# microsoft/VidTok

Hardware: NVIDIA H100
Metric: frames/sec encode+decode, kl_causal_488 17x256x256 (higher is better)
Workload: dtype bf16

## Files before the change

vidtok_b200/csrc/tblock_tc.cu:

```cuda
#include <cuda.h>

#include <cstdio>
#include <cstdlib>
#include <cstring>
#include <string>

#include "common.cuh"
#include "kernels.h"
#include "tc_ptx.cuh"

namespace vt {

namespace {
using namespace tcx;

thread_local std::string g_tb_err;
constexpr int kC = 128;
constexpr int kKc = kC / 64;
constexpr uint32_t kTile = 128 * 128;
constexpr int kHSlots = 3;
constexpr int kConsumerWarps = 8;
constexpr int kProducerWarp = kConsumerWarps;
constexpr int kThreadsTb = (kConsumerWarps + 4) * 32;

struct TbParams {
  int B, T, H, W;
  int BW, BH;
  int tilesW, tilesH;
  long long num_strips;
  int stages;
  const float* bias1;
  const float* bias2;
  const float* g2;
  const float* b2;
  int ln_out, ln_out_silu;
  const float* g3;
  const float* b3;
  const bf16* x;
  bf16* out;
  bf16* out2;
  const bf16* n1;
  int cached_in;
  const bf16* cn1_in;
  const bf16* ch_in;
  bf16* cn1_out;
  bf16* ch_out;
};
struct TbMaps {
  CUtensorMap n1, w1, w2, cn1;
};

__device__ __forceinline__ float quad_sum(float v) {
  v += __shfl_xor_sync(0xffffffffu, v, 1);
  v += __shfl_xor_sync(0xffffffffu, v, 2);
  return v;
}

template <bool kCache>
__global__ void __launch_bounds__(kThreadsTb, 1) tblock_tc_kernel(const __grid_constant__ TbMaps maps, const TbParams p) {
  extern __shared__ uint8_t smem_raw[];
  const uint32_t smem_base = (smem_u32(smem_raw) + 1023u) & ~1023u;
  uint8_t* smem_gen = smem_raw + (smem_base - smem_u32(smem_raw));
  const int warp = threadIdx.x >> 5, lane = threadIdx.x & 31;
  const uint32_t h_base = smem_base;
  const uint32_t ring_base = h_base + kHSlots * kKc * kTile;
  const uint32_t stage_bytes = 2u * kTile;
  const uint32_t bar_base = ring_base + (uint32_t)p.stages * stage_bytes;
  auto full_bar = [&](int s) { return bar_base + 8u * s; };
  auto empty_bar = [&](int s) { return bar_base + 8u * (p.stages + s); };
  float* cst = reinterpret_cast<float*>(smem_gen + (bar_base - smem_base) + 16u * p.stages);

  for (int i = threadIdx.x; i < kC; i += kThreadsTb) {
    cst[i] = p.bias1 ? p.bias1[i] : 0.f;
    cst[kC + i] = 0.5f * p.g2[i];
    cst[2 * kC + i] = 0.5f * p.b2[i];
    cst[3 * kC + i] = p.bias2 ? p.bias2[i] : 0.f;
    const float sc = p.ln_out_silu ? 0.5f : 1.0f;
    cst[4 * kC + i] = p.ln_out ? sc * p.g3[i] : 0.f;
    cst[5 * kC + i] = p.ln_out ? sc * p.b3[i] : 0.f;
  }
  if (threadIdx.x == 0) {
    for (int s = 0; s < p.stages; ++s) { mbar_init(full_bar(s), 1); mbar_init(empty_bar(s), kConsumerWarps); }
    asm volatile("fence.mbarrier_init.release.cluster;" ::: "memory");
  }
  __syncthreads();

  if (warp >= kProducerWarp) {
    asm volatile("setmaxnreg.dec.sync.aligned.u32 40;" ::: "memory");
    if (warp != kProducerWarp) return;
    const bool el = elect_one();
    if (el) { prefetch_tmap(&maps.n1); prefetch_tmap(&maps.w1); prefetch_tmap(&maps.w2); }
    const bool front = kCache && p.cached_in;
    int stage = 0;
    uint32_t phase = 0;
    auto acquire = [&](uint32_t bytes) {
      mbar_wait(empty_bar(stage), phase ^ 1u);
      if (el) mbar_expect_tx(full_bar(stage), bytes);
    };
    auto advance = [&]() { if (++stage == p.stages) { stage = 0; phase ^= 1u; } };
    for (long long strip = blockIdx.x; strip < p.num_strips; strip += gridDim.x) {
      const int tw = (int)(strip % p.tilesW);
      const int th = (int)((strip / p.tilesW) % p.tilesH);
      const int b = (int)(strip / ((long long)p.tilesW * p.tilesH));
      const int w0 = tw * p.BW, h0 = th * p.BH;
      for (int t = 0; t < p.T; ++t) {
        for (int a = 0; a < 3; ++a) {
          const int tv = t - 2 + a;
          if (tv < 0 && !front) continue;
          for (int kc = 0; kc < kKc; ++kc) {
            acquire(2u * kTile);
            if (el) {
              const uint32_t sa = ring_base + stage * stage_bytes;
              if (kCache && tv < 0) tma_load_5d(sa, &maps.cn1, full_bar(stage), kc * 64, w0, h0, tv + 2, b);
              else tma_load_5d(sa, &maps.n1, full_bar(stage), kc * 64, w0, h0, tv, b);
              tma_load_3d(sa + kTile, &maps.w1, full_bar(stage), a * kC + kc * 64, 0, 0);
            }
            advance();
          }
        }
        for (int a = 0; a < 3; ++a) {
          if (t - 2 + a < 0 && !front) continue;
          for (int kc = 0; kc < kKc; ++kc) {
            acquire(kTile);
            if (el) tma_load_3d(ring_base + stage * stage_bytes + kTile, &maps.w2, full_bar(stage), a * kC + kc * 64, 0, 0);
            advance();
          }
        }
      }
    }
    return;
  }

  asm volatile("setmaxnreg.inc.sync.aligned.u32 232;" ::: "memory");
  const int g = warp >> 2, wq = warp & 3;
  const uint32_t hi = desc_hi(1024u);
  float acc[kC / 2];
  int stage = 0, pend_stage = -1;
  uint32_t phase = 0;
  auto release = [&]() {
    if (lane == 0 && pend_stage >= 0) mbar_arrive(empty_bar(pend_stage));
    pend_stage = -1;
  };
  auto kstep = [&](bool a_from_stage, uint32_t h_addr, uint32_t scale) {
    mbar_wait(full_bar(stage), phase);
    const uint32_t sa = ring_base + stage * stage_bytes;
    const uint32_t al = desc_lo(a_from_stage ? sa + (uint32_t)g * 64u * 128u : h_addr), bl = desc_lo(sa + kTile);
    wgmma_fence();
#pragma unroll
    for (uint32_t j = 0; j < 4u; ++j) wgmma_k16<kC, false>(acc, desc(al + 2u * j, hi), desc(bl + 2u * j, hi), j == 0 ? scale : 1u);
    wgmma_commit();
    wgmma_wait<1>();
    release();
    pend_stage = stage;
    if (++stage == p.stages) { stage = 0; phase ^= 1u; }
  };
  auto finish = [&]() {
    wgmma_wait<0>();
    acc_fence(acc);
    release();
  };
  auto wg_sync = [&]() { asm volatile("bar.sync %0, 128;" ::"r"(1 + g) : "memory"); };
  const float* bias1 = cst;
  const float* g2 = cst + kC;
  const float* b2 = cst + 2 * kC;
  const float* bias2 = cst + 3 * kC;
  const float* g3 = cst + 4 * kC;
  const float* b3 = cst + 5 * kC;
  const int cq = 2 * (lane & 3);
  const int rbase = 64 * g + 16 * wq + (lane >> 2);
  const bool front = kCache && p.cached_in;
  const int gtid = threadIdx.x & 127;
  auto slot_of = [&](int tv) { return h_base + (uint32_t)((tv + kHSlots) % kHSlots) * kKc * kTile; };
  auto ring_unit = [&](uint32_t slot, int row, int c) {
    return reinterpret_cast<uint4*>(smem_gen + (slot - smem_base) + (c >> 6) * kTile + row * 128 + ((((c & 63) >> 3) ^ (row & 7)) << 4));
  };

  for (long long strip = blockIdx.x; strip < p.num_strips; strip += gridDim.x) {
    const int tw = (int)(strip % p.tilesW);
    const int th = (int)((strip / p.tilesW) % p.tilesH);
    const int b = (int)(strip / ((long long)p.tilesW * p.tilesH));
    long long pos0[2];
#pragma unroll
    for (int r = 0; r < 2; ++r) {
      const int row = rbase + 8 * r;
      const int h = th * p.BH + row / p.BW, w = tw * p.BW + row % p.BW;
      pos0[r] = (((long long)b * p.T) * p.H + h) * p.W + w;
    }
    const long long frame = (long long)p.H * p.W;
    auto cache_pos = [&](int i, int j, int& row) {
      row = 64 * g + (i >> 4);
      const int h = th * p.BH + row / p.BW, w = tw * p.BW + row % p.BW;
      return ((((long long)b * 2 + j) * p.H + h) * p.W + w) * kC + (i & 15) * 8;
    };
    if (front) {
      wg_sync();
      for (int j = 0; j < 2; ++j)
        for (int i = gtid; i < 64 * 16; i += 128) {
          int row;
          const long long off = cache_pos(i, j, row);
          *ring_unit(slot_of(j - 2), row, (i & 15) * 8) = *reinterpret_cast<const uint4*>(p.ch_in + off);
        }
      fence_async_smem();
      wg_sync();
    }
    for (int t = 0; t < p.T; ++t) {
      uint32_t scale = 0;
      for (int a = 0; a < 3; ++a) {
        if (t - 2 + a < 0 && !front) continue;
        for (int kc = 0; kc < kKc; ++kc) { kstep(true, 0u, scale); scale = 1; }
      }
      finish();
      wg_sync();
      const uint32_t slot = h_base + (uint32_t)(t % kHSlots) * kKc * kTile;
#pragma unroll
      for (int r = 0; r < 2; ++r) {
        float s = 0.f, q = 0.f;
#pragma unroll
        for (int j = 0; j < kC / 8; ++j) {
          const int c = 8 * j + cq;
          const float f0 = acc[4 * j + 2 * r] + bias1[c], f1 = acc[4 * j + 2 * r + 1] + bias1[c + 1];
          s += f0 + f1;
          q = fmaf(f0, f0, q);
          q = fmaf(f1, f1, q);
          const uint32_t kp = pack_bf16x2(f0, f1);
          acc[4 * j + 2 * r] = bf16_lo(kp);
          acc[4 * j + 2 * r + 1] = bf16_hi(kp);
        }
        const float mean = quad_sum(s) * (1.0f / kC);
        float var = fmaf(-mean, mean, quad_sum(q) * (1.0f / kC));
        var = var < 0.f ? 0.f : var;
        const float rstd = rsqrtf(var + 1e-6f);
        const float nmr = -mean * rstd;
        const int row = rbase + 8 * r;
        uint8_t* hrow = smem_gen + (slot - smem_base) + row * 128;
#pragma unroll
        for (int j = 0; j < kC / 8; ++j) {
          const int c = 8 * j + cq;
          float y0 = fmaf(fmaf(acc[4 * j + 2 * r], rstd, nmr), g2[c], b2[c]);
          float y1 = fmaf(fmaf(acc[4 * j + 2 * r + 1], rstd, nmr), g2[c + 1], b2[c + 1]);
          y0 = fmaf(y0, tanh_approx(y0), y0);
          y1 = fmaf(y1, tanh_approx(y1), y1);
          const int cc = c & 63, u = cc >> 3;
          *reinterpret_cast<uint32_t*>(hrow + (c >> 6) * kTile + ((u ^ (row & 7)) << 4) + (cc & 7) * 2) = pack_bf16x2(y0, y1);
        }
      }
      fence_async_smem();
      wg_sync();
      scale = 0;
      for (int a = 0; a < 3; ++a) {
        const int tv = t - 2 + a;
        if (tv < 0 && !front) continue;
        const uint32_t hs = (kCache ? slot_of(tv) : h_base + (uint32_t)(tv % kHSlots) * kKc * kTile) + (uint32_t)g * 64u * 128u;
        for (int kc = 0; kc < kKc; ++kc) { kstep(false, hs + (uint32_t)kc * kTile, scale); scale = 1; }
      }
      finish();
#pragma unroll
      for (int r = 0; r < 2; ++r) {
        const long long off = (pos0[r] + (long long)t * frame) * kC;
        const bf16* xr = p.x + off;
        bf16* orow = p.out + off;
        float s = 0.f, q = 0.f;
#pragma unroll
        for (int j = 0; j < kC / 8; ++j) {
          const int c = 8 * j + cq;
          const uint32_t xw = *reinterpret_cast<const uint32_t*>(xr + c);
          const float f0 = acc[4 * j + 2 * r] + bias2[c] + bf16_lo(xw), f1 = acc[4 * j + 2 * r + 1] + bias2[c + 1] + bf16_hi(xw);
          s += f0 + f1;
          q = fmaf(f0, f0, q);
          q = fmaf(f1, f1, q);
          const uint32_t kp = pack_bf16x2(f0, f1);
          *reinterpret_cast<uint32_t*>(orow + c) = kp;
          acc[4 * j + 2 * r] = bf16_lo(kp);
          acc[4 * j + 2 * r + 1] = bf16_hi(kp);
        }
        if (!p.ln_out) continue;
        const float mean = quad_sum(s) * (1.0f / kC);
        float var = fmaf(-mean, mean, quad_sum(q) * (1.0f / kC));
        var = var < 0.f ? 0.f : var;
        const float rstd = rsqrtf(var + 1e-6f);
        const float nmr = -mean * rstd;
        bf16* o2 = p.out2 + off;
#pragma unroll
        for (int j = 0; j < kC / 8; ++j) {
          const int c = 8 * j + cq;
          float y0 = fmaf(fmaf(acc[4 * j + 2 * r], rstd, nmr), g3[c], b3[c]);
          float y1 = fmaf(fmaf(acc[4 * j + 2 * r + 1], rstd, nmr), g3[c + 1], b3[c + 1]);
          if (p.ln_out_silu) {
            y0 = fmaf(y0, tanh_approx(y0), y0);
            y1 = fmaf(y1, tanh_approx(y1), y1);
          }
          *reinterpret_cast<uint32_t*>(o2 + c) = pack_bf16x2(y0, y1);
        }
      }
    }
    if (kCache) {
      for (int j = 0; j < 2; ++j) {
        const int tv = p.T - 2 + j;
        for (int i = gtid; i < 64 * 16; i += 128) {
          int row;
          const long long off = cache_pos(i, j, row);
          const long long pix = off - (((long long)b * 2 + j) * frame) * kC;
          uint4 hv = make_uint4(0u, 0u, 0u, 0u), nv = hv;
          if (tv >= 0 || front) hv = *ring_unit(slot_of(tv), row, (i & 15) * 8);
          if (tv >= 0) nv = *reinterpret_cast<const uint4*>(p.n1 + (((long long)b * p.T + tv) * frame) * kC + pix);
          else if (front) nv = *reinterpret_cast<const uint4*>(p.cn1_in + (((long long)b * 2 + tv + 2) * frame) * kC + pix);
          *reinterpret_cast<uint4*>(p.ch_out + off) = hv;
          *reinterpret_cast<uint4*>(p.cn1_out + off) = nv;
        }
      }
    }
  }
}

typedef CUresult (*EncodeTiledFn)(CUtensorMap*, CUtensorMapDataType, cuuint32_t, void*, const cuuint64_t*,
                                  const cuuint64_t*, const cuuint32_t*, const cuuint32_t*, CUtensorMapInterleave,
                                  CUtensorMapSwizzle, CUtensorMapL2promotion, CUtensorMapFloatOOBfill);
EncodeTiledFn tb_get_encode() {
  static EncodeTiledFn fn = nullptr;
  static bool tried = false;
  if (!tried) {
    tried = true;
    void* f = nullptr;
    cudaDriverEntryPointQueryResult q;
    if (cudaGetDriverEntryPoint("cuTensorMapEncodeTiled", &f, cudaEnableDefault, &q) == cudaSuccess && q == cudaDriverEntryPointSuccess)
      fn = (EncodeTiledFn)f;
  }
  return fn;
}

bool strip_box(int H, int W, int& BW, int& BH) {
  for (int bw = 128; bw >= 1; bw >>= 1) {
    if (W % bw != 0) continue;
    const int bh = 128 / bw;
    if (bh <= 256 && H % bh == 0) { BW = bw; BH = bh; return true; }
  }
  return false;
}
}

const char* tblock_tc_last_error() { return g_tb_err.c_str(); }

bool tblock_tc_supported(int B, int T, int H, int W, int C, bool planning) {
  g_tb_err.clear();
  static int env = -1;
  if (env < 0) { const char* e = getenv("VT_TBLOCK"); env = e ? atoi(e) : 1; }
  if (!env) { g_tb_err = "disabled (VT_TBLOCK=0)"; return false; }
  if (C != kC) { g_tb_err = "C != 128"; return false; }
  if (B <= 0 || T <= 0) { g_tb_err = "empty"; return false; }
  int BW, BH;
  if (!strip_box(H, W, BW, BH)) { g_tb_err = "H x W not tileable by a 128-position box"; return false; }
  if (!planning && !tb_get_encode()) { g_tb_err = "cuTensorMapEncodeTiled unavailable"; return false; }
  return true;
}

cudaError_t launch_tblock_tc(const bf16* n1, const bf16* x, const bf16* w1, const float* bias1, const float* gamma2,
                             const float* beta2, const bf16* w2, const float* bias2, bf16* out, bf16* out2,
                             const float* gamma_out, const float* beta_out, bool out_silu, int B, int T, int H, int W,
                             cudaStream_t s, const TbCache* cache) {
  g_tb_err.clear();
  EncodeTiledFn enc = tb_get_encode();
  if (!enc) { g_tb_err = "cuTensorMapEncodeTiled unavailable"; return cudaErrorNotSupported; }
  TbParams p;
  memset(&p, 0, sizeof(p));
  if (!strip_box(H, W, p.BW, p.BH)) { g_tb_err = "H x W not tileable"; return cudaErrorInvalidValue; }
  p.B = B; p.T = T; p.H = H; p.W = W;
  p.tilesW = W / p.BW; p.tilesH = H / p.BH;
  p.num_strips = (long long)B * p.tilesH * p.tilesW;
  p.bias1 = bias1; p.bias2 = bias2; p.g2 = gamma2; p.b2 = beta2;
  p.ln_out = (out2 && gamma_out && beta_out) ? 1 : 0;
  p.ln_out_silu = out_silu ? 1 : 0;
  p.g3 = gamma_out; p.b3 = beta_out;
  p.x = x; p.out = out; p.out2 = out2;
  if (cache) {
    if (!cache->n1_out || !cache->h_out || (!cache->n1_in != !cache->h_in)) { g_tb_err = "cache: both outputs, and both or no inputs"; return cudaErrorInvalidValue; }
    p.n1 = n1;
    p.cached_in = cache->n1_in ? 1 : 0;
    p.cn1_in = cache->n1_in; p.ch_in = cache->h_in; p.cn1_out = cache->n1_out; p.ch_out = cache->h_out;
  }
  const size_t fixed = 1024 + (size_t)kHSlots * kKc * kTile + 6 * kC * 4;
  const size_t budget = 225 * 1024;
  int stages = (int)((budget - fixed) / (2 * kTile + 16));
  if (stages > 4) stages = 4;
  p.stages = stages;
  const size_t smem = fixed + (size_t)stages * (2 * kTile + 16);
  TbMaps maps;
  {
    cuuint64_t dims[5] = {(cuuint64_t)kC, (cuuint64_t)W, (cuuint64_t)H, (cuuint64_t)T, (cuuint64_t)B};
    cuuint64_t strides[4] = {(cuuint64_t)kC * 2, (cuuint64_t)W * kC * 2, (cuuint64_t)H * W * kC * 2, (cuuint64_t)T * H * W * kC * 2};
    cuuint32_t box[5] = {64, (cuuint32_t)p.BW, (cuuint32_t)p.BH, 1, 1};
    cuuint32_t es[5] = {1, 1, 1, 1, 1};
    CUresult r = enc(&maps.n1, CU_TENSOR_MAP_DATA_TYPE_BFLOAT16, 5, const_cast<bf16*>(n1), dims, strides, box, es, CU_TENSOR_MAP_INTERLEAVE_NONE,
                     CU_TENSOR_MAP_SWIZZLE_128B, CU_TENSOR_MAP_L2_PROMOTION_L2_256B, CU_TENSOR_MAP_FLOAT_OOB_FILL_NONE);
    if (r != CUDA_SUCCESS) { g_tb_err = "cuTensorMapEncodeTiled(n1) failed: " + std::to_string((int)r); return cudaErrorInvalidValue; }
    maps.cn1 = maps.n1;
    if (p.cached_in) {
      dims[3] = 2;
      strides[3] = 2ull * H * W * kC * 2;
      r = enc(&maps.cn1, CU_TENSOR_MAP_DATA_TYPE_BFLOAT16, 5, const_cast<bf16*>(p.cn1_in), dims, strides, box, es, CU_TENSOR_MAP_INTERLEAVE_NONE,
              CU_TENSOR_MAP_SWIZZLE_128B, CU_TENSOR_MAP_L2_PROMOTION_L2_256B, CU_TENSOR_MAP_FLOAT_OOB_FILL_NONE);
      if (r != CUDA_SUCCESS) { g_tb_err = "cuTensorMapEncodeTiled(n1 cache) failed: " + std::to_string((int)r); return cudaErrorInvalidValue; }
    }
  }
  for (int i = 0; i < 2; ++i) {
    cuuint64_t dims[3] = {(cuuint64_t)(3 * kC), (cuuint64_t)kC, 1};
    cuuint64_t strides[2] = {(cuuint64_t)(3 * kC) * 2, (cuuint64_t)(3 * kC) * kC * 2};
    cuuint32_t box[3] = {64, (cuuint32_t)kC, 1};
    cuuint32_t es[3] = {1, 1, 1};
    CUresult r = enc(i ? &maps.w2 : &maps.w1, CU_TENSOR_MAP_DATA_TYPE_BFLOAT16, 3, const_cast<bf16*>(i ? w2 : w1), dims, strides, box, es,
                     CU_TENSOR_MAP_INTERLEAVE_NONE, CU_TENSOR_MAP_SWIZZLE_128B, CU_TENSOR_MAP_L2_PROMOTION_L2_256B,
                     CU_TENSOR_MAP_FLOAT_OOB_FILL_NONE);
    if (r != CUDA_SUCCESS) { g_tb_err = "cuTensorMapEncodeTiled(weights) failed: " + std::to_string((int)r); return cudaErrorInvalidValue; }
  }
  static bool attr[64] = {false};
  static int sms[64] = {0};
  int dev = 0;
  cudaGetDevice(&dev);
  if (dev < 0 || dev >= 64) return cudaErrorInvalidDevice;
  if (!attr[dev]) {
    for (auto k : {tblock_tc_kernel<false>, tblock_tc_kernel<true>}) {
      cudaError_t e = cudaFuncSetAttribute(k, cudaFuncAttributeMaxDynamicSharedMemorySize, (int)(227 * 1024));
      if (e != cudaSuccess) { g_tb_err = "cudaFuncSetAttribute(smem)"; return e; }
    }
    attr[dev] = true;
    cudaDeviceGetAttribute(&sms[dev], cudaDevAttrMultiProcessorCount, dev);
    if (sms[dev] <= 0) sms[dev] = 132;
  }
  const unsigned grid = (unsigned)(p.num_strips < sms[dev] ? p.num_strips : sms[dev]);
  const double M = (double)B * T * H * W;
  char det[96] = "";
  if (prof_enabled()) snprintf(det, sizeof(det), cache ? "strip %dx%d T%d ln_out%d cache%d" : "strip %dx%d T%d ln_out%d", p.BH, p.BW, T,
                               p.ln_out, p.cached_in);
  ProfScope _ps("tblock_tc", 2.0 * 2.0 * M * 3 * kC * kC, 2.0 * M * kC * (3.0 + (p.ln_out ? 1.0 : 0.0)), s, det);
  if (cache) tblock_tc_kernel<true><<<grid, kThreadsTb, smem, s>>>(maps, p);
  else tblock_tc_kernel<false><<<grid, kThreadsTb, smem, s>>>(maps, p);
  count_launch();
  return cudaGetLastError();
}

}
```

vidtok_b200/csrc/tc_ptx.cuh:

```cuda
#pragma once
#include <cuda.h>
#include <cuda_bf16.h>
#include <cuda_fp16.h>
#include <stdint.h>

namespace vt {
namespace tcx {
__device__ __forceinline__ uint32_t smem_u32(const void* p) { return (uint32_t)__cvta_generic_to_shared(p); }

__device__ __forceinline__ void mbar_init(uint32_t bar, uint32_t count) {
  asm volatile("mbarrier.init.shared::cta.b64 [%0], %1;" ::"r"(bar), "r"(count) : "memory");
}
__device__ __forceinline__ void mbar_expect_tx(uint32_t bar, uint32_t bytes) {
  asm volatile("mbarrier.arrive.expect_tx.shared::cta.b64 _, [%0], %1;" ::"r"(bar), "r"(bytes) : "memory");
}
__device__ __forceinline__ void mbar_arrive(uint32_t bar) {
  asm volatile("mbarrier.arrive.shared::cta.b64 _, [%0];" ::"r"(bar) : "memory");
}
__device__ __forceinline__ bool mbar_try_wait(uint32_t bar, uint32_t parity) {
  uint32_t ok;
  asm volatile(
      "{\n\t"
      ".reg .pred p;\n\t"
      "mbarrier.try_wait.parity.shared::cta.b64 p, [%1], %2;\n\t"
      "selp.u32 %0, 1, 0, p;\n\t"
      "}"
      : "=r"(ok)
      : "r"(bar), "r"(parity)
      : "memory");
  return ok != 0;
}
__device__ __forceinline__ void mbar_wait(uint32_t bar, uint32_t parity) {
  if (mbar_try_wait(bar, parity)) return;
  const long long t0 = clock64();
  while (!mbar_try_wait(bar, parity)) {
    if (clock64() - t0 > 8000000000LL) __trap();
  }
}
__device__ __forceinline__ void tma_load_5d(uint32_t dst, const CUtensorMap* map, uint32_t bar, int c0, int c1, int c2,
                                            int c3, int c4) {
  asm volatile(
      "cp.async.bulk.tensor.5d.shared::cluster.global.mbarrier::complete_tx::bytes [%0], [%1, {%3, %4, %5, %6, %7}], [%2];"
      ::"r"(dst), "l"(map), "r"(bar), "r"(c0), "r"(c1), "r"(c2), "r"(c3), "r"(c4)
      : "memory");
}
__device__ __forceinline__ void tma_load_3d(uint32_t dst, const CUtensorMap* map, uint32_t bar, int c0, int c1, int c2) {
  asm volatile(
      "cp.async.bulk.tensor.3d.shared::cluster.global.mbarrier::complete_tx::bytes [%0], [%1, {%3, %4, %5}], [%2];"
      ::"r"(dst), "l"(map), "r"(bar), "r"(c0), "r"(c1), "r"(c2)
      : "memory");
}
__device__ __forceinline__ void fence_async_smem() { asm volatile("fence.proxy.async.shared::cta;" ::: "memory"); }
__device__ __forceinline__ void named_bar_sync(uint32_t id, uint32_t threads) {
  asm volatile("bar.sync %0, %1;" ::"r"(id), "r"(threads) : "memory");
}
__device__ __forceinline__ void named_bar_arrive(uint32_t id, uint32_t threads) {
  asm volatile("bar.arrive %0, %1;" ::"r"(id), "r"(threads) : "memory");
}
__device__ __forceinline__ void prefetch_tmap(const CUtensorMap* map) {
  asm volatile("prefetch.tensormap [%0];" ::"l"(map) : "memory");
}
__device__ __forceinline__ bool elect_one() {
  uint32_t pred;
  asm volatile(
      "{\n\t"
      ".reg .pred P1;\n\t"
      "elect.sync _|P1, 0xffffffff;\n\t"
      "selp.u32 %0, 1, 0, P1;\n\t"
      "}"
      : "=r"(pred));
  return pred != 0;
}

__device__ __forceinline__ void wgmma_fence() { asm volatile("wgmma.fence.sync.aligned;" ::: "memory"); }
__device__ __forceinline__ void wgmma_commit() { asm volatile("wgmma.commit_group.sync.aligned;" ::: "memory"); }
template <int kPending>
__device__ __forceinline__ void wgmma_wait() { asm volatile("wgmma.wait_group.sync.aligned %0;" ::"n"(kPending) : "memory"); }
template <int R>
__device__ __forceinline__ void acc_fence(float (&d)[R]) {
#pragma unroll
  for (int i = 0; i < R; ++i) asm volatile("" : "+f"(d[i])::"memory");
}

__device__ __forceinline__ uint32_t desc_lo(uint32_t saddr) { return ((saddr & 0x3FFFFu) >> 4) | (1u << 16); }
__device__ __forceinline__ uint32_t desc_hi(uint32_t sbo) { return (sbo >> 4) | (1u << 30); }
__device__ __forceinline__ uint64_t desc(uint32_t lo, uint32_t hi) { return ((uint64_t)hi << 32) | lo; }

__device__ __forceinline__ void wgmma_32_bf16(float (&d)[16], uint64_t da, uint64_t db, uint32_t scale_d) {
  asm volatile(
      "{\n\t.reg .pred p;\n\t"
      "setp.ne.b32 p, %18, 0;\n\t"
      "wgmma.mma_async.sync.aligned.m64n32k16.f32.bf16.bf16 "
      "{"
      "%0, %1, %2, %3, %4, %5, %6, %7, %8, %9, %10, %11, %12, %13, %14, %15"
      "}, %16, %17, p, 1, 1, 0, 0;\n\t}"
      : "+f"(d[0]), "+f"(d[1]), "+f"(d[2]), "+f"(d[3]), "+f"(d[4]), "+f"(d[5]), "+f"(d[6]), "+f"(d[7]),
        "+f"(d[8]), "+f"(d[9]), "+f"(d[10]), "+f"(d[11]), "+f"(d[12]), "+f"(d[13]), "+f"(d[14]), "+f"(d[15])
      : "l"(da), "l"(db), "r"(scale_d));
}
__device__ __forceinline__ void wgmma_32_f16(float (&d)[16], uint64_t da, uint64_t db, uint32_t scale_d) {
  asm volatile(
      "{\n\t.reg .pred p;\n\t"
      "setp.ne.b32 p, %18, 0;\n\t"
      "wgmma.mma_async.sync.aligned.m64n32k16.f32.f16.f16 "
      "{"
      "%0, %1, %2, %3, %4, %5, %6, %7, %8, %9, %10, %11, %12, %13, %14, %15"
      "}, %16, %17, p, 1, 1, 0, 0;\n\t}"
      : "+f"(d[0]), "+f"(d[1]), "+f"(d[2]), "+f"(d[3]), "+f"(d[4]), "+f"(d[5]), "+f"(d[6]), "+f"(d[7]),
        "+f"(d[8]), "+f"(d[9]), "+f"(d[10]), "+f"(d[11]), "+f"(d[12]), "+f"(d[13]), "+f"(d[14]), "+f"(d[15])
      : "l"(da), "l"(db), "r"(scale_d));
}
__device__ __forceinline__ void wgmma_64_bf16(float (&d)[32], uint64_t da, uint64_t db, uint32_t scale_d) {
  asm volatile(
      "{\n\t.reg .pred p;\n\t"
      "setp.ne.b32 p, %34, 0;\n\t"
      "wgmma.mma_async.sync.aligned.m64n64k16.f32.bf16.bf16 "
      "{"
      "%0, %1, %2, %3, %4, %5, %6, %7, %8, %9, %10, %11, %12, %13, %14, %15, "
      "%16, %17, %18, %19, %20, %21, %22, %23, %24, %25, %26, %27, %28, %29, %30, %31"
      "}, %32, %33, p, 1, 1, 0, 0;\n\t}"
      : "+f"(d[0]), "+f"(d[1]), "+f"(d[2]), "+f"(d[3]), "+f"(d[4]), "+f"(d[5]), "+f"(d[6]), "+f"(d[7]),
        "+f"(d[8]), "+f"(d[9]), "+f"(d[10]), "+f"(d[11]), "+f"(d[12]), "+f"(d[13]), "+f"(d[14]), "+f"(d[15]),
        "+f"(d[16]), "+f"(d[17]), "+f"(d[18]), "+f"(d[19]), "+f"(d[20]), "+f"(d[21]), "+f"(d[22]), "+f"(d[23]),
        "+f"(d[24]), "+f"(d[25]), "+f"(d[26]), "+f"(d[27]), "+f"(d[28]), "+f"(d[29]), "+f"(d[30]), "+f"(d[31])
      : "l"(da), "l"(db), "r"(scale_d));
}
__device__ __forceinline__ void wgmma_64_f16(float (&d)[32], uint64_t da, uint64_t db, uint32_t scale_d) {
  asm volatile(
      "{\n\t.reg .pred p;\n\t"
      "setp.ne.b32 p, %34, 0;\n\t"
      "wgmma.mma_async.sync.aligned.m64n64k16.f32.f16.f16 "
      "{"
      "%0, %1, %2, %3, %4, %5, %6, %7, %8, %9, %10, %11, %12, %13, %14, %15, "
      "%16, %17, %18, %19, %20, %21, %22, %23, %24, %25, %26, %27, %28, %29, %30, %31"
      "}, %32, %33, p, 1, 1, 0, 0;\n\t}"
      : "+f"(d[0]), "+f"(d[1]), "+f"(d[2]), "+f"(d[3]), "+f"(d[4]), "+f"(d[5]), "+f"(d[6]), "+f"(d[7]),
        "+f"(d[8]), "+f"(d[9]), "+f"(d[10]), "+f"(d[11]), "+f"(d[12]), "+f"(d[13]), "+f"(d[14]), "+f"(d[15]),
        "+f"(d[16]), "+f"(d[17]), "+f"(d[18]), "+f"(d[19]), "+f"(d[20]), "+f"(d[21]), "+f"(d[22]), "+f"(d[23]),
        "+f"(d[24]), "+f"(d[25]), "+f"(d[26]), "+f"(d[27]), "+f"(d[28]), "+f"(d[29]), "+f"(d[30]), "+f"(d[31])
      : "l"(da), "l"(db), "r"(scale_d));
}
__device__ __forceinline__ void wgmma_128_bf16(float (&d)[64], uint64_t da, uint64_t db, uint32_t scale_d) {
  asm volatile(
      "{\n\t.reg .pred p;\n\t"
      "setp.ne.b32 p, %66, 0;\n\t"
      "wgmma.mma_async.sync.aligned.m64n128k16.f32.bf16.bf16 "
      "{"
      "%0, %1, %2, %3, %4, %5, %6, %7, %8, %9, %10, %11, %12, %13, %14, %15, "
      "%16, %17, %18, %19, %20, %21, %22, %23, %24, %25, %26, %27, %28, %29, %30, %31, "
      "%32, %33, %34, %35, %36, %37, %38, %39, %40, %41, %42, %43, %44, %45, %46, %47, "
      "%48, %49, %50, %51, %52, %53, %54, %55, %56, %57, %58, %59, %60, %61, %62, %63"
      "}, %64, %65, p, 1, 1, 0, 0;\n\t}"
      : "+f"(d[0]), "+f"(d[1]), "+f"(d[2]), "+f"(d[3]), "+f"(d[4]), "+f"(d[5]), "+f"(d[6]), "+f"(d[7]),
        "+f"(d[8]), "+f"(d[9]), "+f"(d[10]), "+f"(d[11]), "+f"(d[12]), "+f"(d[13]), "+f"(d[14]), "+f"(d[15]),
        "+f"(d[16]), "+f"(d[17]), "+f"(d[18]), "+f"(d[19]), "+f"(d[20]), "+f"(d[21]), "+f"(d[22]), "+f"(d[23]),
        "+f"(d[24]), "+f"(d[25]), "+f"(d[26]), "+f"(d[27]), "+f"(d[28]), "+f"(d[29]), "+f"(d[30]), "+f"(d[31]),
        "+f"(d[32]), "+f"(d[33]), "+f"(d[34]), "+f"(d[35]), "+f"(d[36]), "+f"(d[37]), "+f"(d[38]), "+f"(d[39]),
        "+f"(d[40]), "+f"(d[41]), "+f"(d[42]), "+f"(d[43]), "+f"(d[44]), "+f"(d[45]), "+f"(d[46]), "+f"(d[47]),
        "+f"(d[48]), "+f"(d[49]), "+f"(d[50]), "+f"(d[51]), "+f"(d[52]), "+f"(d[53]), "+f"(d[54]), "+f"(d[55]),
        "+f"(d[56]), "+f"(d[57]), "+f"(d[58]), "+f"(d[59]), "+f"(d[60]), "+f"(d[61]), "+f"(d[62]), "+f"(d[63])
      : "l"(da), "l"(db), "r"(scale_d));
}
__device__ __forceinline__ void wgmma_128_f16(float (&d)[64], uint64_t da, uint64_t db, uint32_t scale_d) {
  asm volatile(
      "{\n\t.reg .pred p;\n\t"
      "setp.ne.b32 p, %66, 0;\n\t"
      "wgmma.mma_async.sync.aligned.m64n128k16.f32.f16.f16 "
      "{"
      "%0, %1, %2, %3, %4, %5, %6, %7, %8, %9, %10, %11, %12, %13, %14, %15, "
      "%16, %17, %18, %19, %20, %21, %22, %23, %24, %25, %26, %27, %28, %29, %30, %31, "
      "%32, %33, %34, %35, %36, %37, %38, %39, %40, %41, %42, %43, %44, %45, %46, %47, "
      "%48, %49, %50, %51, %52, %53, %54, %55, %56, %57, %58, %59, %60, %61, %62, %63"
      "}, %64, %65, p, 1, 1, 0, 0;\n\t}"
      : "+f"(d[0]), "+f"(d[1]), "+f"(d[2]), "+f"(d[3]), "+f"(d[4]), "+f"(d[5]), "+f"(d[6]), "+f"(d[7]),
        "+f"(d[8]), "+f"(d[9]), "+f"(d[10]), "+f"(d[11]), "+f"(d[12]), "+f"(d[13]), "+f"(d[14]), "+f"(d[15]),
        "+f"(d[16]), "+f"(d[17]), "+f"(d[18]), "+f"(d[19]), "+f"(d[20]), "+f"(d[21]), "+f"(d[22]), "+f"(d[23]),
        "+f"(d[24]), "+f"(d[25]), "+f"(d[26]), "+f"(d[27]), "+f"(d[28]), "+f"(d[29]), "+f"(d[30]), "+f"(d[31]),
        "+f"(d[32]), "+f"(d[33]), "+f"(d[34]), "+f"(d[35]), "+f"(d[36]), "+f"(d[37]), "+f"(d[38]), "+f"(d[39]),
        "+f"(d[40]), "+f"(d[41]), "+f"(d[42]), "+f"(d[43]), "+f"(d[44]), "+f"(d[45]), "+f"(d[46]), "+f"(d[47]),
        "+f"(d[48]), "+f"(d[49]), "+f"(d[50]), "+f"(d[51]), "+f"(d[52]), "+f"(d[53]), "+f"(d[54]), "+f"(d[55]),
        "+f"(d[56]), "+f"(d[57]), "+f"(d[58]), "+f"(d[59]), "+f"(d[60]), "+f"(d[61]), "+f"(d[62]), "+f"(d[63])
      : "l"(da), "l"(db), "r"(scale_d));
}
__device__ __forceinline__ void wgmma_256_bf16(float (&d)[128], uint64_t da, uint64_t db, uint32_t scale_d) {
  asm volatile(
      "{\n\t.reg .pred p;\n\t"
      "setp.ne.b32 p, %130, 0;\n\t"
      "wgmma.mma_async.sync.aligned.m64n256k16.f32.bf16.bf16 "
      "{"
      "%0, %1, %2, %3, %4, %5, %6, %7, %8, %9, %10, %11, %12, %13, %14, %15, "
      "%16, %17, %18, %19, %20, %21, %22, %23, %24, %25, %26, %27, %28, %29, %30, %31, "
      "%32, %33, %34, %35, %36, %37, %38, %39, %40, %41, %42, %43, %44, %45, %46, %47, "
      "%48, %49, %50, %51, %52, %53, %54, %55, %56, %57, %58, %59, %60, %61, %62, %63, "
      "%64, %65, %66, %67, %68, %69, %70, %71, %72, %73, %74, %75, %76, %77, %78, %79, "
      "%80, %81, %82, %83, %84, %85, %86, %87, %88, %89, %90, %91, %92, %93, %94, %95, "
      "%96, %97, %98, %99, %100, %101, %102, %103, %104, %105, %106, %107, %108, %109, %110, %111, "
      "%112, %113, %114, %115, %116, %117, %118, %119, %120, %121, %122, %123, %124, %125, %126, %127"
      "}, %128, %129, p, 1, 1, 0, 0;\n\t}"
      : "+f"(d[0]), "+f"(d[1]), "+f"(d[2]), "+f"(d[3]), "+f"(d[4]), "+f"(d[5]), "+f"(d[6]), "+f"(d[7]),
        "+f"(d[8]), "+f"(d[9]), "+f"(d[10]), "+f"(d[11]), "+f"(d[12]), "+f"(d[13]), "+f"(d[14]), "+f"(d[15]),
        "+f"(d[16]), "+f"(d[17]), "+f"(d[18]), "+f"(d[19]), "+f"(d[20]), "+f"(d[21]), "+f"(d[22]), "+f"(d[23]),
        "+f"(d[24]), "+f"(d[25]), "+f"(d[26]), "+f"(d[27]), "+f"(d[28]), "+f"(d[29]), "+f"(d[30]), "+f"(d[31]),
        "+f"(d[32]), "+f"(d[33]), "+f"(d[34]), "+f"(d[35]), "+f"(d[36]), "+f"(d[37]), "+f"(d[38]), "+f"(d[39]),
        "+f"(d[40]), "+f"(d[41]), "+f"(d[42]), "+f"(d[43]), "+f"(d[44]), "+f"(d[45]), "+f"(d[46]), "+f"(d[47]),
        "+f"(d[48]), "+f"(d[49]), "+f"(d[50]), "+f"(d[51]), "+f"(d[52]), "+f"(d[53]), "+f"(d[54]), "+f"(d[55]),
        "+f"(d[56]), "+f"(d[57]), "+f"(d[58]), "+f"(d[59]), "+f"(d[60]), "+f"(d[61]), "+f"(d[62]), "+f"(d[63]),
        "+f"(d[64]), "+f"(d[65]), "+f"(d[66]), "+f"(d[67]), "+f"(d[68]), "+f"(d[69]), "+f"(d[70]), "+f"(d[71]),
        "+f"(d[72]), "+f"(d[73]), "+f"(d[74]), "+f"(d[75]), "+f"(d[76]), "+f"(d[77]), "+f"(d[78]), "+f"(d[79]),
        "+f"(d[80]), "+f"(d[81]), "+f"(d[82]), "+f"(d[83]), "+f"(d[84]), "+f"(d[85]), "+f"(d[86]), "+f"(d[87]),
        "+f"(d[88]), "+f"(d[89]), "+f"(d[90]), "+f"(d[91]), "+f"(d[92]), "+f"(d[93]), "+f"(d[94]), "+f"(d[95]),
        "+f"(d[96]), "+f"(d[97]), "+f"(d[98]), "+f"(d[99]), "+f"(d[100]), "+f"(d[101]), "+f"(d[102]), "+f"(d[103]),
        "+f"(d[104]), "+f"(d[105]), "+f"(d[106]), "+f"(d[107]), "+f"(d[108]), "+f"(d[109]), "+f"(d[110]), "+f"(d[111]),
        "+f"(d[112]), "+f"(d[113]), "+f"(d[114]), "+f"(d[115]), "+f"(d[116]), "+f"(d[117]), "+f"(d[118]), "+f"(d[119]),
        "+f"(d[120]), "+f"(d[121]), "+f"(d[122]), "+f"(d[123]), "+f"(d[124]), "+f"(d[125]), "+f"(d[126]), "+f"(d[127])
      : "l"(da), "l"(db), "r"(scale_d));
}
__device__ __forceinline__ void wgmma_256_f16(float (&d)[128], uint64_t da, uint64_t db, uint32_t scale_d) {
  asm volatile(
      "{\n\t.reg .pred p;\n\t"
      "setp.ne.b32 p, %130, 0;\n\t"
      "wgmma.mma_async.sync.aligned.m64n256k16.f32.f16.f16 "
      "{"
      "%0, %1, %2, %3, %4, %5, %6, %7, %8, %9, %10, %11, %12, %13, %14, %15, "
      "%16, %17, %18, %19, %20, %21, %22, %23, %24, %25, %26, %27, %28, %29, %30, %31, "
      "%32, %33, %34, %35, %36, %37, %38, %39, %40, %41, %42, %43, %44, %45, %46, %47, "
      "%48, %49, %50, %51, %52, %53, %54, %55, %56, %57, %58, %59, %60, %61, %62, %63, "
      "%64, %65, %66, %67, %68, %69, %70, %71, %72, %73, %74, %75, %76, %77, %78, %79, "
      "%80, %81, %82, %83, %84, %85, %86, %87, %88, %89, %90, %91, %92, %93, %94, %95, "
      "%96, %97, %98, %99, %100, %101, %102, %103, %104, %105, %106, %107, %108, %109, %110, %111, "
      "%112, %113, %114, %115, %116, %117, %118, %119, %120, %121, %122, %123, %124, %125, %126, %127"
      "}, %128, %129, p, 1, 1, 0, 0;\n\t}"
      : "+f"(d[0]), "+f"(d[1]), "+f"(d[2]), "+f"(d[3]), "+f"(d[4]), "+f"(d[5]), "+f"(d[6]), "+f"(d[7]),
        "+f"(d[8]), "+f"(d[9]), "+f"(d[10]), "+f"(d[11]), "+f"(d[12]), "+f"(d[13]), "+f"(d[14]), "+f"(d[15]),
        "+f"(d[16]), "+f"(d[17]), "+f"(d[18]), "+f"(d[19]), "+f"(d[20]), "+f"(d[21]), "+f"(d[22]), "+f"(d[23]),
        "+f"(d[24]), "+f"(d[25]), "+f"(d[26]), "+f"(d[27]), "+f"(d[28]), "+f"(d[29]), "+f"(d[30]), "+f"(d[31]),
        "+f"(d[32]), "+f"(d[33]), "+f"(d[34]), "+f"(d[35]), "+f"(d[36]), "+f"(d[37]), "+f"(d[38]), "+f"(d[39]),
        "+f"(d[40]), "+f"(d[41]), "+f"(d[42]), "+f"(d[43]), "+f"(d[44]), "+f"(d[45]), "+f"(d[46]), "+f"(d[47]),
        "+f"(d[48]), "+f"(d[49]), "+f"(d[50]), "+f"(d[51]), "+f"(d[52]), "+f"(d[53]), "+f"(d[54]), "+f"(d[55]),
        "+f"(d[56]), "+f"(d[57]), "+f"(d[58]), "+f"(d[59]), "+f"(d[60]), "+f"(d[61]), "+f"(d[62]), "+f"(d[63]),
        "+f"(d[64]), "+f"(d[65]), "+f"(d[66]), "+f"(d[67]), "+f"(d[68]), "+f"(d[69]), "+f"(d[70]), "+f"(d[71]),
        "+f"(d[72]), "+f"(d[73]), "+f"(d[74]), "+f"(d[75]), "+f"(d[76]), "+f"(d[77]), "+f"(d[78]), "+f"(d[79]),
        "+f"(d[80]), "+f"(d[81]), "+f"(d[82]), "+f"(d[83]), "+f"(d[84]), "+f"(d[85]), "+f"(d[86]), "+f"(d[87]),
        "+f"(d[88]), "+f"(d[89]), "+f"(d[90]), "+f"(d[91]), "+f"(d[92]), "+f"(d[93]), "+f"(d[94]), "+f"(d[95]),
        "+f"(d[96]), "+f"(d[97]), "+f"(d[98]), "+f"(d[99]), "+f"(d[100]), "+f"(d[101]), "+f"(d[102]), "+f"(d[103]),
        "+f"(d[104]), "+f"(d[105]), "+f"(d[106]), "+f"(d[107]), "+f"(d[108]), "+f"(d[109]), "+f"(d[110]), "+f"(d[111]),
        "+f"(d[112]), "+f"(d[113]), "+f"(d[114]), "+f"(d[115]), "+f"(d[116]), "+f"(d[117]), "+f"(d[118]), "+f"(d[119]),
        "+f"(d[120]), "+f"(d[121]), "+f"(d[122]), "+f"(d[123]), "+f"(d[124]), "+f"(d[125]), "+f"(d[126]), "+f"(d[127])
      : "l"(da), "l"(db), "r"(scale_d));
}

template <int N, bool kF16>
__device__ __forceinline__ void wgmma_k16(float (&d)[N / 2], uint64_t da, uint64_t db, uint32_t scale_d) {
  if constexpr (N == 32) { if constexpr (kF16) wgmma_32_f16(d, da, db, scale_d); else wgmma_32_bf16(d, da, db, scale_d); }
  else if constexpr (N == 64) { if constexpr (kF16) wgmma_64_f16(d, da, db, scale_d); else wgmma_64_bf16(d, da, db, scale_d); }
  else if constexpr (N == 128) { if constexpr (kF16) wgmma_128_f16(d, da, db, scale_d); else wgmma_128_bf16(d, da, db, scale_d); }
  else { static_assert(N == 256, "N tile"); if constexpr (kF16) wgmma_256_f16(d, da, db, scale_d); else wgmma_256_bf16(d, da, db, scale_d); }
}

__device__ __forceinline__ void unpack8(const uint4& u, float (&f)[8]) {
  const __nv_bfloat162* h = reinterpret_cast<const __nv_bfloat162*>(&u);
#pragma unroll
  for (int i = 0; i < 4; ++i) {
    f[2 * i] = __low2float(h[i]);
    f[2 * i + 1] = __high2float(h[i]);
  }
}
__device__ __forceinline__ uint32_t pack_bf16x2(float lo, float hi) {
  uint32_t r;
  asm("cvt.rn.bf16x2.f32 %0, %1, %2;" : "=r"(r) : "f"(hi), "f"(lo));
  return r;
}
__device__ __forceinline__ float tanh_approx(float x) { float t; asm("tanh.approx.f32 %0, %1;" : "=f"(t) : "f"(x)); return t; }
__device__ __forceinline__ uint32_t pack_f16x2(float lo, float hi) {
  lo = fminf(fmaxf(lo, -65504.0f), 65504.0f);
  hi = fminf(fmaxf(hi, -65504.0f), 65504.0f);
  uint32_t r;
  asm("cvt.rn.f16x2.f32 %0, %1, %2;" : "=r"(r) : "f"(hi), "f"(lo));
  return r;
}
__device__ __forceinline__ float f16_lo(uint32_t w) { return __half2float(__ushort_as_half((unsigned short)(w & 0xFFFFu))); }
__device__ __forceinline__ float f16_hi(uint32_t w) { return __half2float(__ushort_as_half((unsigned short)(w >> 16))); }
__device__ __forceinline__ void unpack8h(const uint4& u, float (&f)[8]) {
  const __half2* h = reinterpret_cast<const __half2*>(&u);
#pragma unroll
  for (int i = 0; i < 4; ++i) {
    const float2 v = __half22float2(h[i]);
    f[2 * i] = v.x;
    f[2 * i + 1] = v.y;
  }
}
__device__ __forceinline__ float bf16_lo(uint32_t w) { float f; asm("mov.b32 %0, %1;" : "=f"(f) : "r"(w << 16)); return f; }
__device__ __forceinline__ float bf16_hi(uint32_t w) { float f; asm("mov.b32 %0, %1;" : "=f"(f) : "r"(w & 0xFFFF0000u)); return f; }

}
}
```

Baseline: 438.6.

## Load residual input and store block output via TMA through a free h slot

The residual input x is now loaded by TMA into a free shared-memory h-ring slot, issued during the second GEMM so the load overlaps compute. The epilogue reads and writes the residual through that swizzled slot, and the finished tile goes back to global memory with a TMA bulk store. This replaces per-thread scattered 4-byte global loads and stores in the epilogue. In exchange it adds mbarriers, bulk-group waits, an extra workgroup sync and careful slot-reuse ordering, all of which add synchronisation cost and raise correctness risk.

```diff
diff --git a/vidtok_b200/csrc/tblock_tc.cu b/vidtok_b200/csrc/tblock_tc.cu
--- a/vidtok_b200/csrc/tblock_tc.cu
+++ b/vidtok_b200/csrc/tblock_tc.cu
@@ -48,6 +48,7 @@
 };
 struct TbMaps {
   CUtensorMap n1, w1, w2, cn1;
+  CUtensorMap x, out;
 };
 
 __device__ __forceinline__ float quad_sum(float v) {
@@ -68,7 +69,8 @@
   const uint32_t bar_base = ring_base + (uint32_t)p.stages * stage_bytes;
   auto full_bar = [&](int s) { return bar_base + 8u * s; };
   auto empty_bar = [&](int s) { return bar_base + 8u * (p.stages + s); };
-  float* cst = reinterpret_cast<float*>(smem_gen + (bar_base - smem_base) + 16u * p.stages);
+  auto x_bar = [&](int g) { return bar_base + 16u * p.stages + 8u * g; };
+  float* cst = reinterpret_cast<float*>(smem_gen + (bar_base - smem_base) + 16u * p.stages + 16u);
 
   for (int i = threadIdx.x; i < kC; i += kThreadsTb) {
     cst[i] = p.bias1 ? p.bias1[i] : 0.f;
@@ -81,6 +83,7 @@
   }
   if (threadIdx.x == 0) {
     for (int s = 0; s < p.stages; ++s) { mbar_init(full_bar(s), 1); mbar_init(empty_bar(s), kConsumerWarps); }
+    for (int g = 0; g < 2; ++g) mbar_init(x_bar(g), 1);
     asm volatile("fence.mbarrier_init.release.cluster;" ::: "memory");
   }
   __syncthreads();
@@ -136,7 +139,7 @@
   const uint32_t hi = desc_hi(1024u);
   float acc[kC / 2];
   int stage = 0, pend_stage = -1;
-  uint32_t phase = 0;
+  uint32_t phase = 0, xphase = 0;
   auto release = [&]() {
     if (lane == 0 && pend_stage >= 0) mbar_arrive(empty_bar(pend_stage));
     pend_stage = -1;
@@ -193,6 +196,7 @@
       return ((((long long)b * 2 + j) * p.H + h) * p.W + w) * kC + (i & 15) * 8;
     };
     if (front) {
+      if (gtid == 0) bulk_wait_read<0>();
       wg_sync();
       for (int j = 0; j < 2; ++j)
         for (int i = gtid; i < 64 * 16; i += 128) {
@@ -203,6 +207,13 @@
       fence_async_smem();
       wg_sync();
     }
+    const int box_w = tw * p.BW + (64 * g) % p.BW, box_h = th * p.BH + (64 * g) / p.BW;
+    auto x_load = [&](int t) {
+      if (gtid != 0) return;
+      const uint32_t dst = slot_of(t - 2) + (uint32_t)g * 64u * 128u;
+      mbar_expect_tx(x_bar(g), (uint32_t)kKc * 64u * 128u);
+      for (int kc = 0; kc < kKc; ++kc) tma_load_5d(dst + (uint32_t)kc * kTile, &maps.x, x_bar(g), kc * 64, box_w, box_h, t, b);
+    };
     for (int t = 0; t < p.T; ++t) {
       uint32_t scale = 0;
       for (int a = 0; a < 3; ++a) {
@@ -210,6 +221,7 @@
         for (int kc = 0; kc < kKc; ++kc) { kstep(true, 0u, scale); scale = 1; }
       }
       finish();
+      if (gtid == 0) bulk_wait_read<0>();
       wg_sync();
       const uint32_t slot = h_base + (uint32_t)(t % kHSlots) * kKc * kTile;
 #pragma unroll
@@ -246,30 +258,42 @@
       }
       fence_async_smem();
       wg_sync();
+      const bool tap0 = t >= 2 || front;
+      if (!tap0) x_load(t);
       scale = 0;
+      int s2 = 0;
       for (int a = 0; a < 3; ++a) {
         const int tv = t - 2 + a;
         if (tv < 0 && !front) continue;
         const uint32_t hs = (kCache ? slot_of(tv) : h_base + (uint32_t)(tv % kHSlots) * kKc * kTile) + (uint32_t)g * 64u * 128u;
-        for (int kc = 0; kc < kKc; ++kc) { kstep(false, hs + (uint32_t)kc * kTile, scale); scale = 1; }
+        for (int kc = 0; kc < kKc; ++kc) {
+          kstep(false, hs + (uint32_t)kc * kTile, scale);
+          scale = 1;
+          if (++s2 == kKc + 1 && tap0) { wg_sync(); x_load(t); }
+        }
       }
       finish();
+      mbar_wait(x_bar(g), xphase);
+      xphase ^= 1u;
+      const uint32_t xslot = slot_of(t - 2);
 #pragma unroll
       for (int r = 0; r < 2; ++r) {
         const long long off = (pos0[r] + (long long)t * frame) * kC;
-        const bf16* xr = p.x + off;
-        bf16* orow = p.out + off;
+        const int row = rbase + 8 * r;
+        uint8_t* xrow = smem_gen + (xslot - smem_base) + row * 128;
         float s = 0.f, q = 0.f;
 #pragma unroll
         for (int j = 0; j < kC / 8; ++j) {
           const int c = 8 * j + cq;
-          const uint32_t xw = *reinterpret_cast<const uint32_t*>(xr + c);
+          const int cc = c & 63, u = cc >> 3;
+          uint32_t* xo = reinterpret_cast<uint32_t*>(xrow + (c >> 6) * kTile + ((u ^ (row & 7)) << 4) + (cc & 7) * 2);
+          const uint32_t xw = *xo;
           const float f0 = acc[4 * j + 2 * r] + bias2[c] + bf16_lo(xw), f1 = acc[4 * j + 2 * r + 1] + bias2[c + 1] + bf16_hi(xw);
           s += f0 + f1;
           q = fmaf(f0, f0, q);
           q = fmaf(f1, f1, q);
           const uint32_t kp = pack_bf16x2(f0, f1);
-          *reinterpret_cast<uint32_t*>(orow + c) = kp;
+          *xo = kp;
           acc[4 * j + 2 * r] = bf16_lo(kp);
           acc[4 * j + 2 * r + 1] = bf16_hi(kp);
         }
@@ -291,6 +315,13 @@
           }
           *reinterpret_cast<uint32_t*>(o2 + c) = pack_bf16x2(y0, y1);
         }
+      }
+      fence_async_smem();
+      wg_sync();
+      if (gtid == 0) {
+        for (int kc = 0; kc < kKc; ++kc)
+          tma_store_5d(&maps.out, xslot + (uint32_t)g * 64u * 128u + (uint32_t)kc * kTile, kc * 64, box_w, box_h, t, b);
+        bulk_commit();
       }
     }
     if (kCache) {
@@ -310,6 +341,7 @@
       }
     }
   }
+  if (gtid == 0) bulk_wait<0>();
 }
 
 typedef CUresult (*EncodeTiledFn)(CUtensorMap*, CUtensorMapDataType, cuuint32_t, void*, const cuuint64_t*,
@@ -377,7 +409,7 @@
     p.cached_in = cache->n1_in ? 1 : 0;
     p.cn1_in = cache->n1_in; p.ch_in = cache->h_in; p.cn1_out = cache->n1_out; p.ch_out = cache->h_out;
   }
-  const size_t fixed = 1024 + (size_t)kHSlots * kKc * kTile + 6 * kC * 4;
+  const size_t fixed = 1024 + (size_t)kHSlots * kKc * kTile + 16 + 6 * kC * 4;
   const size_t budget = 225 * 1024;
   int stages = (int)((budget - fixed) / (2 * kTile + 16));
   if (stages > 4) stages = 4;
@@ -393,6 +425,13 @@
                      CU_TENSOR_MAP_SWIZZLE_128B, CU_TENSOR_MAP_L2_PROMOTION_L2_256B, CU_TENSOR_MAP_FLOAT_OOB_FILL_NONE);
     if (r != CUDA_SUCCESS) { g_tb_err = "cuTensorMapEncodeTiled(n1) failed: " + std::to_string((int)r); return cudaErrorInvalidValue; }
     maps.cn1 = maps.n1;
+    const int bw = p.BW < 64 ? p.BW : 64;
+    cuuint32_t box64[5] = {64, (cuuint32_t)bw, (cuuint32_t)(64 / bw), 1, 1};
+    for (int i = 0; i < 2; ++i) {
+      r = enc(i ? &maps.out : &maps.x, CU_TENSOR_MAP_DATA_TYPE_BFLOAT16, 5, i ? (void*)out : const_cast<bf16*>(x), dims, strides, box64, es,
+              CU_TENSOR_MAP_INTERLEAVE_NONE, CU_TENSOR_MAP_SWIZZLE_128B, CU_TENSOR_MAP_L2_PROMOTION_L2_256B, CU_TENSOR_MAP_FLOAT_OOB_FILL_NONE);
+      if (r != CUDA_SUCCESS) { g_tb_err = "cuTensorMapEncodeTiled(x / out) failed: " + std::to_string((int)r); return cudaErrorInvalidValue; }
+    }
     if (p.cached_in) {
       dims[3] = 2;
       strides[3] = 2ull * H * W * kC * 2;
diff --git a/vidtok_b200/csrc/tc_ptx.cuh b/vidtok_b200/csrc/tc_ptx.cuh
--- a/vidtok_b200/csrc/tc_ptx.cuh
+++ b/vidtok_b200/csrc/tc_ptx.cuh
@@ -50,6 +50,16 @@
       ::"r"(dst), "l"(map), "r"(bar), "r"(c0), "r"(c1), "r"(c2)
       : "memory");
 }
+__device__ __forceinline__ void tma_store_5d(const CUtensorMap* map, uint32_t src, int c0, int c1, int c2, int c3, int c4) {
+  asm volatile("cp.async.bulk.tensor.5d.global.shared::cta.bulk_group [%0, {%2, %3, %4, %5, %6}], [%1];"
+               ::"l"(map), "r"(src), "r"(c0), "r"(c1), "r"(c2), "r"(c3), "r"(c4)
+               : "memory");
+}
+__device__ __forceinline__ void bulk_commit() { asm volatile("cp.async.bulk.commit_group;" ::: "memory"); }
+template <int kPending>
+__device__ __forceinline__ void bulk_wait_read() { asm volatile("cp.async.bulk.wait_group.read %0;" ::"n"(kPending) : "memory"); }
+template <int kPending>
+__device__ __forceinline__ void bulk_wait() { asm volatile("cp.async.bulk.wait_group %0;" ::"n"(kPending) : "memory"); }
 __device__ __forceinline__ void fence_async_smem() { asm volatile("fence.proxy.async.shared::cta;" ::: "memory"); }
 __device__ __forceinline__ void named_bar_sync(uint32_t id, uint32_t threads) {
   asm volatile("bar.sync %0, %1;" ::"r"(id), "r"(threads) : "memory");
```

New measurement: 459.4 (median of 6 runs). 4.7% higher.
